# JVBSouza/descriptools

Hardware: AMD Instinct MI355X
Metric: Mcells/s full descriptor chain (higher is better)
Workload: dtype f32; 1 GPU; 16384x16384 synthetic tilted-integer-fBm DEM per GPU, full chain (d8, flowacc, river mask, flowhand/HAND with fused GFI + ln(hl/H), fused slope+TI+MTI, downslope), device-resident; global_dem=16384x16384, river_threshold_cells=524288

## Files before the change

### descriptools_amd/csrc/dt_tiles.hip

```cpp
#include "dt_common.h"
#include "dt_kernels.h"
#include "dt_math.h"

#define TW 64
#define TH 64
#define NT (TW * TH)
#define PS (2 * TW + 2 * (TH - 2))
#define CPT (NT / 256)

#define NX_SINK 0xFFFFu
#define NX_EXIT 0xFFFEu
#define NX_REXIT 0xFFFDu
#define X_NONE 0xFFFFu

__device__ __forceinline__ int dt_slot_of(int ly, int lx) {
  if (ly == 0) return lx;
  if (ly == TH - 1) return TW + lx;
  if (lx == 0) return 2 * TW + (ly - 1);
  if (lx == TW - 1) return 2 * TW + (TH - 2) + (ly - 1);
  return -1;
}
__device__ __forceinline__ void dt_cell_of_slot(int s, int &ly, int &lx) {
  if (s < TW) { ly = 0; lx = s; }
  else if (s < 2 * TW) { ly = TH - 1; lx = s - TW; }
// ... 1201 lines not shown
  if (NODES && threadIdx.x < PS) {
    int ly, lx;
    dt_cell_of_slot(threadIdx.x, ly, lx);
    unsigned long long s = s_st[ly * TW + lx];
    uint32_t ptr = (uint32_t)(s >> 32), nd = (uint32_t)((s >> 16) & 0xFFFFu);
    uint32_t ncf = (uint32_t)(s & 0xFFFFu), nc = ncf & 0x7FFFu;
    uint32_t kind = (ptr >> 12) & 7u, f = ptr & 0xFFFu;
    int fy = (int)f / TW, fx = (int)f % TW;
    unsigned long long o = fht_pack(FHT_DEAD, 0, FHT_DONE);
    if (!(ncf & FHT_DONE)) {
    } else if (kind == K_RIVER) {
      o = fht_pack((uint32_t)((y0 + fy) * w.W + x0 + fx), nd, nc | FHT_DONE);
    } else if (kind == K_EXIT || kind == K_REXIT) {
      int dy, dx;
      dt_d8_delta(s_fdr[f], dy, dx);
      bool diag = dy != 0 && dx != 0;
      uint32_t node = kind == K_EXIT ? dt_node_of(y0 + fy + dy, x0 + fx + dx, tiles_x)
                                     : nnodes + (uint32_t)dt_perim_index(w.H, w.W, y0 + fy, x0 + fx);
      o = fht_pack(node, nd + (diag ? 1u : 0u), nc + (diag ? 0u : 1u));
    }
    nodes[(size_t)tile * PS + threadIdx.x] = o;
  }
  unsigned long long wv[CPT];
  int wide = 0;
#pragma unroll
  for (int j = 0; j < CPT; j++) {
    wv[j] = s_st[threadIdx.x + 256 * j];
    wide |= (((uint32_t)wv[j] & 0x7FFFu) > 255u || ((uint32_t)(wv[j] >> 16) & 0xFFFFu) > 255u) ? 1 : 0;
  }
  wide = __syncthreads_or(wide);
  if (threadIdx.x == 0) cache_wide[tile] = (uint8_t)wide;
  if (wide) {
#pragma unroll
    for (int j = 0; j < CPT; j++) cache[(size_t)tile * NT + threadIdx.x + 256 * j] = wv[j];
  } else {
    uint32_t *c32 = reinterpret_cast<uint32_t *>(cache + (size_t)tile * NT);
#pragma unroll
    for (int j = 0; j < CPT; j++) c32[threadIdx.x + 256 * j] = fh_cache_pack(wv[j]);
  }
  __syncthreads();
}
__global__ __launch_bounds__(256) void k_fh_tile1(const uint8_t *__restrict__ fdr,
                                                 const int8_t *__restrict__ river, DtWin w, int tiles_x,
                                                 uint32_t nnodes, unsigned long long *__restrict__ nodes,
                                                 unsigned long long *__restrict__ cache,
                                                 uint8_t *__restrict__ cache_wide, int only_marked, int ntiles) {
  __shared__ __attribute__((aligned(16))) uint8_t s_fdr[NT];
  __shared__ uint8_t s_halo[2 * (TW + 2) + 2 * TH];
  __shared__ __attribute__((aligned(16))) unsigned long long s_st[NT];
  for (int tile = (int)blockIdx.x; tile < ntiles; tile += (int)gridDim.x) {
    if (only_marked && cache_wide[tile] != 2) continue;
    fh_tile1_tile<true>(s_fdr, s_halo, s_st, tile, fdr, river, w, tiles_x, nnodes, nodes, cache, cache_wide);
  }
}
__global__ __launch_bounds__(256) void k_fh_tile1_marked(const uint8_t *__restrict__ fdr,
                                                        const int8_t *__restrict__ river, DtWin w, int tiles_x,
                                                        uint32_t nnodes, unsigned long long *__restrict__ nodes,
                                                        unsigned long long *__restrict__ cache,
                                                        uint8_t *cache_wide, int ntiles) {
  __shared__ __attribute__((aligned(16))) uint8_t s_fdr[NT];
  __shared__ uint8_t s_halo[2 * (TW + 2) + 2 * TH];
  __shared__ __attribute__((aligned(16))) unsigned long long s_st[NT];
  __shared__ uint8_t s_flag[256];
  const int base = (int)blockIdx.x * 256, mine = base + (int)threadIdx.x;
  const uint8_t flag = mine < ntiles ? cache_wide[mine] : (uint8_t)0;
  s_flag[threadIdx.x] = flag;
  if (!__syncthreads_or(flag == 2)) return;
  for (int i = 0; i < 256; i++)
    if (s_flag[i] == 2)
      fh_tile1_tile<false>(s_fdr, s_halo, s_st, base + i, fdr, river, w, tiles_x, nnodes, nodes, cache, cache_wide);
}

#define FN_CNT 0x3FFFFu
#define FN_DONE 0x40000u
#define FN_LOW 0x7FFFFu
#define FN_OVF 0x20100u
#define FN_PTR_SH 19
__device__ __forceinline__ uint32_t fh_lut_entry(uint32_t code) {
  if (!dt_d8_valid(code)) return 0u;
  int dy, dx;
  dt_d8_delta(code, dy, dx);
  return ((uint32_t)(dy * TW + dx) << FN_PTR_SH) + ((dy != 0 && dx != 0) ? (1u << 9) : 1u);
}
__device__ __forceinline__ bool fh_tile1n_solve(uint8_t *s_fdr, uint32_t *s_w, uint8_t *s_kind, int *s_ovf_p,
                                                const uint32_t *s_lut, const uint32_t (&riv4)[NT / 4 / 256],
                                                const DtWin &w, int y0, int x0, uint2 (&own)[CPT / 2]) {
#define s_ovf (*s_ovf_p)
  const bool interior = dt_tile_interior(w, y0, x0);
  const uint32_t lx0 = (4u * threadIdx.x) & 63u;
#pragma unroll
  for (int u = 0; u < NT / 4 / 256; u++) {
    const int c0 = 4 * (threadIdx.x + 256 * u);
    const uint32_t codes = *reinterpret_cast<const uint32_t *>(&s_fdr[c0]);
    uint32_t wd[4], kinds = 0;
#pragma unroll
    for (int k = 0; k < 4; k++) {
      const int c = c0 + k;
      const uint32_t code = (codes >> (8 * k)) & 0xFFu, cw = (uint32_t)c << FN_PTR_SH;
      const bool is_river = ((riv4[u] >> (8 * k)) & 0xFFu) == 1u;
      uint32_t word = cw | FN_DONE, kind = K_DEAD;
      if (interior) {
        const uint32_t wn = cw + s_lut[code];
        if (code != 0u) {
          if (is_river) {
            kind = K_RIVER;
          } else if (wn & FN_CNT) {
            const bool out = (int32_t)wn < 0 || (((wn >> FN_PTR_SH) & 63u) - (lx0 + (uint32_t)k - 1u)) > 2u;
            if (out) kind = K_EXIT;
            else word = wn;
          }
        }
      } else {
        const int ly = c / TW, lx = c % TW;
        const int y = y0 + ly, x = x0 + lx;
        if (y < w.H && x < w.W && code != 0u) {
          if (is_river) {
            kind = K_RIVER;
          } else if (dt_d8_valid(code)) {
            int dy, dx;
            dt_d8_delta(code, dy, dx);
            uint32_t ny = (uint32_t)(ly + dy), nx = (uint32_t)(lx + dx);
            bool in_tile = ny < (uint32_t)TH && nx < (uint32_t)TW;
            if (dt_in_global(w, y + dy, x + dx)) {
              if (!dt_in_core(w, y + dy, x + dx)) kind = K_REXIT;
              else if (!in_tile) kind = K_EXIT;
              else word = ((ny * TW + nx) << FN_PTR_SH) | ((dy != 0 && dx != 0) ? (1u << 9) : 1u);
            }
          }
        }
      }
      wd[k] = word;
      kinds |= kind << (8 * k);
    }
    *reinterpret_cast<uint4 *>(&s_w[c0]) = make_uint4(wd[0], wd[1], wd[2], wd[3]);
    *reinterpret_cast<uint32_t *>(&s_kind[c0]) = kinds;
  }
  __syncthreads();
  uint2 *s_w2 = reinterpret_cast<uint2 *>(s_w);
#pragma unroll
  for (int j = 0; j < CPT / 2; j++) own[j] = s_w2[threadIdx.x + 256 * j];
  for (int round = 0; round < 13; round++) {
    int changed = 0;
    uint32_t ovf = 0;
#pragma unroll
    for (int j = 0; j < CPT / 2; j++) {
      int c2 = threadIdx.x + 256 * j;
      uint2 v = own[j];
      bool dx = (v.x & FN_DONE) != 0u, dy = (v.y & FN_DONE) != 0u;
      if (dx && dy) continue;
      if (!dx) {
        v.x = s_w[v.x >> FN_PTR_SH] + (v.x & FN_CNT);
        if (!(v.x & (FN_DONE | FN_OVF))) v.x = s_w[v.x >> FN_PTR_SH] + (v.x & FN_CNT);
        ovf |= v.x & FN_OVF;
      }
      if (!dy) {
        v.y = s_w[v.y >> FN_PTR_SH] + (v.y & FN_CNT);
        if (!(v.y & (FN_DONE | FN_OVF))) v.y = s_w[v.y >> FN_PTR_SH] + (v.y & FN_CNT);
        ovf |= v.y & FN_OVF;
      }
      own[j] = v;
      s_w2[c2] = v;
      changed |= ((v.x & v.y & FN_DONE) == 0u) ? 1 : 0;
    }
    if (ovf) s_ovf = 1;
    if (!__syncthreads_or(changed)) break;
    if (s_ovf) break;
  }
  return !s_ovf;
#undef s_ovf
}
__device__ __forceinline__ uint32_t fh_narrow_word(uint32_t v, uint32_t c, const uint8_t *s_kind) {
  uint32_t f = v >> FN_PTR_SH, kind = s_kind[f];
  if (!(v & FN_DONE)) { f = c; kind = K_DEAD; v = 0; }
  return f | (kind << 12) | (((v >> 9) & 0xFFu) << 15) | ((v & 0xFFu) << 23);
}
__device__ __forceinline__ void fh_tile1n_body(uint8_t *s_fdr, uint32_t *s_w, uint8_t *s_kind, int *s_ovf_p,
                                               const uint32_t *s_lut, const uint32_t (&riv4)[NT / 4 / 256],
                                               const DtWin &w, int tile, int tiles_x, int y0, int x0, uint32_t nnodes,
                                               unsigned long long *__restrict__ nodes,
                                               unsigned long long *__restrict__ cache,
                                               uint8_t *__restrict__ cache_wide) {
  uint2 own[CPT / 2];
  if (!fh_tile1n_solve(s_fdr, s_w, s_kind, s_ovf_p, s_lut, riv4, w, y0, x0, own)) {
    if (threadIdx.x == 0) cache_wide[tile] = 2;
    return;
  }
  uint2 *s_w2 = reinterpret_cast<uint2 *>(s_w);
  auto narrow = [&](uint32_t v, uint32_t c) -> uint32_t { return fh_narrow_word(v, c, s_kind); };
#pragma unroll
  for (int j = 0; j < CPT / 2; j++) {
    const int c2 = threadIdx.x + 256 * j;
    s_w2[c2] = make_uint2(narrow(own[j].x, 2u * (uint32_t)c2), narrow(own[j].y, 2u * (uint32_t)c2 + 1u));
  }
  if (threadIdx.x == 0) cache_wide[tile] = 0;
  __syncthreads();
  uint32_t *c32 = reinterpret_cast<uint32_t *>(cache + (size_t)tile * NT);
#pragma unroll
  for (int u = 0; u < NT / 4 / 256; u++) {
    int c = 4 * (threadIdx.x + 256 * u);
    *reinterpret_cast<uint4 *>(c32 + c) = *reinterpret_cast<const uint4 *>(&s_w[c]);
  }
  if (threadIdx.x < PS) {
    int ly, lx;
    dt_cell_of_slot(threadIdx.x, ly, lx);
    unsigned long long sw = fh_cache_unpack(s_w[ly * TW + lx]);
    uint32_t ptr = (uint32_t)(sw >> 32), nd = (uint32_t)((sw >> 16) & 0xFFFFu), nc = (uint32_t)sw & 0x7FFFu;
    uint32_t kind = (ptr >> 12) & 7u, f = ptr & 0xFFFu;
    int fy = (int)f / TW, fx = (int)f % TW;
    unsigned long long o = fht_pack(FHT_DEAD, 0, FHT_DONE);
    if (kind == K_RIVER) {
      o = fht_pack((uint32_t)((y0 + fy) * w.W + x0 + fx), nd, nc | FHT_DONE);
    } else if (kind == K_EXIT || kind == K_REXIT) {
      int dy, dx;
      dt_d8_delta(s_fdr[f], dy, dx);
      bool diag = dy != 0 && dx != 0;
      uint32_t node = kind == K_EXIT ? dt_node_of(y0 + fy + dy, x0 + fx + dx, tiles_x)
                                     : nnodes + (uint32_t)dt_perim_index(w.H, w.W, y0 + fy, x0 + fx);
      o = fht_pack(node, nd + (diag ? 1u : 0u), nc + (diag ? 0u : 1u));
    }
    nodes[(size_t)tile * PS + threadIdx.x] = o;
  }
}

#define NX_RIVER 0xFFFCu
#define FH_SOLVE_LATER 3
__device__ __forceinline__ void fh_walk_body(const uint16_t *s_nxt, const uint8_t *__restrict__ fdr, bool fed, const DtWin &w,
                                             int tile, int tiles_x, int y0, int x0,
                                             unsigned long long *__restrict__ nodes,
                                             uint8_t *__restrict__ cache_wide) {
  constexpr uint32_t PW = TW + 4, NTP = TH * PW;
  if (threadIdx.x == 0) cache_wide[tile] = (uint8_t)FH_SOLVE_LATER;
  if (threadIdx.x >= PS) return;
  unsigned long long o = fht_pack(FHT_DEAD, 0, FHT_DONE);
  if (fed) {
    int ly, lx;
    dt_cell_of_slot(threadIdx.x, ly, lx);
    uint32_t c = (uint32_t)ly * PW + (uint32_t)lx, nc = 0, nd = 0;
    uint32_t n = 0;
    for (int it = 0; it < NT; it++) {
      n = s_nxt[c];
      if (n >= NTP) break;
      const uint32_t d = n > c ? n - c : c - n;
      if (d == 1u || d == PW) nc++;
      else nd++;
      c = n;
    }
    if (n == NX_RIVER || n == NX_EXIT) {
      const int fy = (int)(c / PW), fx = (int)(c % PW);
      const uint32_t code = fdr[(long long)(y0 + fy) * w.ld + x0 + fx];
      if (n == NX_EXIT) {
        int dy, dx;
        dt_d8_delta(code, dy, dx);
        const bool diag = dy != 0 && dx != 0;
        o = fht_pack(dt_node_of(y0 + fy + dy, x0 + fx + dx, tiles_x), nd + (diag ? 1u : 0u), nc + (diag ? 0u : 1u));
      } else if (code != 0u) {
// ... 111 lines not shown
  uint8_t k = (uint8_t)K_DEAD;
  int32_t r = -1;
  float z = DT_NODATA;
  long long a = 0;
  if (ncf & FHT_DONE) {
    if (ptr != FHT_DEAD) {
      k = (uint8_t)K_RIVER;
      r = (int32_t)ptr;
      long long o = (long long)(ptr / (uint32_t)w.W) * w.ld + (ptr % (uint32_t)w.W);
      if (dem) z = dem[o];
      if (acc32) a = (long long)acc32[o];
    }
  } else if (ptr >= nnodes) {
    k = (uint8_t)K_REXIT;
    r = (int32_t)(ptr - nnodes);
  }
  kind[i] = k;
  ref[i] = r;
  nc[i] = (int32_t)(ncf & 0x7FFFu);
  nd[i] = (int32_t)((s >> 16) & 0xFFFFu);
  zr[i] = z;
  ar[i] = a;
}

__global__ __launch_bounds__(256) void k_fh_ghost_set(unsigned long long *__restrict__ nodes, uint32_t nnodes,
                                                     int64_t P, const uint8_t *__restrict__ res_ok,
                                                     const int32_t *__restrict__ res_nc,
                                                     const int32_t *__restrict__ res_nd) {
  int64_t i = (int64_t)blockIdx.x * 256 + threadIdx.x;
  if (i >= P) return;
  unsigned long long o = fht_pack(FHT_DEAD, 0, FHT_DONE);
  if (res_ok[i]) o = fht_pack(FHT_REMOTE | (uint32_t)i, (uint32_t)res_nd[i], (uint32_t)res_nc[i] | FHT_DONE);
  nodes[nnodes + i] = o;
}

struct FhGfi {
  float *gfi, *lnhlh;
  double expo, c0;
  const DtLogEntry *tab;
};
struct FhRemote {
  const long long *gidx;
  const float *zr;
  const long long *ar;
};
template <typename AccT>
struct FhPay;
template <>
struct FhPay<int32_t> {
  unsigned long long v[PS];
  __device__ __forceinline__ void set(int i, float z, int32_t a) {
    v[i] = ((unsigned long long)(uint32_t)a << 32) | (unsigned long long)__float_as_uint(z);
  }
  __device__ __forceinline__ void get(int i, float &z, int32_t &a) const {
    const unsigned long long p = v[i];
    z = __uint_as_float((uint32_t)p);
    a = (int32_t)(uint32_t)(p >> 32);
  }
};
template <>
struct FhPay<long long> {
  long long av[PS];
  float zv[PS];
  __device__ __forceinline__ void set(int i, float z, long long a) {
    av[i] = a;
    zv[i] = z;
  }
  __device__ __forceinline__ void get(int i, float &z, long long &a) const {
    z = zv[i];
    a = av[i];
  }
};

typedef float fh_v4f __attribute__((ext_vector_type(4)));
typedef int fh_v4i __attribute__((ext_vector_type(4)));
__device__ __forceinline__ void fh_store4(float *p, float a, float b, float c, float d) {
  fh_v4f v = {a, b, c, d};
  __builtin_nontemporal_store(v, reinterpret_cast<fh_v4f *>(p));
}
__device__ __forceinline__ void fh_store4(int32_t *p, int32_t a, int32_t b, int32_t c, int32_t d) {
  fh_v4i v = {a, b, c, d};
  __builtin_nontemporal_store(v, reinterpret_cast<fh_v4i *>(p));
}
typedef long long fh_v2l __attribute__((ext_vector_type(2)));
__device__ __forceinline__ void fh_store4(long long *p, long long a, long long b, long long c, long long d) {
  fh_v2l v0 = {a, b}, v1 = {c, d};
  __builtin_nontemporal_store(v0, reinterpret_cast<fh_v2l *>(p));
  __builtin_nontemporal_store(v1, reinterpret_cast<fh_v2l *>(p + 2));
}

struct FhSolveLds {
  uint8_t *fdr;
  uint32_t *w;
  uint8_t *kind;
  uint32_t *lut;
  int *ovf;
  double *term;
};
template <bool RANKED, int VH, typename AccT, bool SOLVE>
__device__ __forceinline__ bool fh_tile3_tile(unsigned long long *s_x, FhPay<AccT> &s_pay, DtLogEntry *s_tab,
                                              const FhSolveLds &L, const int8_t *__restrict__ river, int tile,
                                              const uint8_t *__restrict__ fdr, const float *__restrict__ dem,
                                              const AccT *__restrict__ acc32, const DtWin &w, int tiles_x,
                                              uint32_t nnodes, const unsigned long long *__restrict__ nodes,
                                              const unsigned long long *__restrict__ cache, bool wide,
                                              const FhRemote &rem, double px, float *__restrict__ fdist,
                                              int32_t *__restrict__ idx32, long long *__restrict__ idx64,
                                              float *__restrict__ hand, AccT *__restrict__ a_river,
                                              const FhGfi &G) {
  const int ty = tile / tiles_x, tx = tile - ty * tiles_x;
  const int y0 = ty * TH, x0 = tx * TW;
  const bool vec = x0 + TW <= w.W && (w.ld & 3) == 0 && (!dem || ((uintptr_t)dem & 15) == 0) &&
                   (!fdist || ((uintptr_t)fdist & 15) == 0) && (!idx32 || ((uintptr_t)idx32 & 15) == 0) &&
                   (!idx64 || ((uintptr_t)idx64 & 15) == 0) && (!hand || ((uintptr_t)hand & 15) == 0) &&
                   (!a_river || ((uintptr_t)a_river & 15) == 0) &&
                   (!G.gfi || ((((uintptr_t)G.gfi | (uintptr_t)G.lnhlh | (uintptr_t)acc32) & 15) == 0));
  [[maybe_unused]] auto load_z4 = [&](int u) -> float4 {
    const int c = 4 * (threadIdx.x + 256 * u), y = y0 + c / TW;
    float4 z = make_float4(DT_NODATA, DT_NODATA, DT_NODATA, DT_NODATA);
    if (dem && y < w.H) z = *reinterpret_cast<const float4 *>(dem + (long long)y * w.ld + x0 + c % TW);
    return z;
  };
  [[maybe_unused]] auto load_f4 = [&](int u) -> int4 {
    const int c = 4 * (threadIdx.x + 256 * u), y = y0 + c / TW;
    int4 f = make_int4(0, 0, 0, 0);
    if (G.gfi && y < w.H) f = *reinterpret_cast<const int4 *>(acc32 + (long long)y * w.ld + x0 + c % TW);
    return f;
  };
  float4 z4_first = make_float4(DT_NODATA, DT_NODATA, DT_NODATA, DT_NODATA);
  int4 f4_first = make_int4(0, 0, 0, 0);
  int slot_ly = 0, slot_lx = 0;
  if (threadIdx.x < PS) dt_cell_of_slot(threadIdx.x, slot_ly, slot_lx);
  uint32_t slot_code = 0;
  bool has_river = true;
  if (SOLVE) {
    const uint4 v_fdr = dt_tile_fetch16(fdr, w, y0, x0);
    const uint4 v_riv = dt_tile_fetch16(reinterpret_cast<const uint8_t *>(river), w, y0, x0);
    if (vec) {
      z4_first = load_z4(0);
      f4_first = load_f4(0);
    }
    dt_tile_put16(L.fdr, v_fdr);
    dt_tile_put16(L.kind, v_riv);
    L.lut[threadIdx.x] = fh_lut_entry(threadIdx.x);
    if (threadIdx.x == 0) *L.ovf = 0;
    has_river = __syncthreads_or((v_riv.x | v_riv.y | v_riv.z | v_riv.w) != 0u) != 0;
    if (threadIdx.x < PS) slot_code = L.fdr[slot_ly * TW + slot_lx];
    uint32_t riv4[NT / 4 / 256];
#pragma unroll
    for (int u = 0; u < NT / 4 / 256; u++) riv4[u] = *reinterpret_cast<const uint32_t *>(&L.kind[4 * (threadIdx.x + 256 * u)]);
    uint2 own[CPT / 2];
    if (!fh_tile1n_solve(L.fdr, L.w, L.kind, L.ovf, L.lut, riv4, w, y0, x0, own)) return false;
  }
  auto solved = [&](uint32_t v, int c) -> uint32_t { return fh_narrow_word(v, (uint32_t)c, L.kind); };
  if (threadIdx.x < PS) {
    const int ly = slot_ly, lx = slot_lx;
    int f = ly * TW + lx;
    bool ex, rex;
    if (SOLVE) {
      const uint32_t v = L.w[f];
      const bool self = (v & FN_DONE) != 0u && (v >> FN_PTR_SH) == (uint32_t)f;
      const uint32_t kind = L.kind[f];
      ex = self && kind == K_EXIT;
      rex = self && kind == K_REXIT;
    } else {
      const uint32_t sp = (uint32_t)(fh_cache_get(cache, wide, tile, f) >> 32);
      ex = sp == ((uint32_t)f | (K_EXIT << 12));
      rex = sp == ((uint32_t)f | (K_REXIT << 12));
    }
    unsigned long long o = fht_pack(FHT_DEAD, 0, FHT_DONE);
    float zr = DT_NODATA;
    AccT ar = -100;
    if (ex || rex) {
      int dy, dx;
      dt_d8_delta(SOLVE ? slot_code : (uint32_t)fdr[(long long)(y0 + ly) * w.ld + x0 + lx], dy, dx);
      size_t node = ex ? (size_t)dt_node_of(y0 + ly + dy, x0 + lx + dx, tiles_x)
                       : (size_t)nnodes + (size_t)dt_perim_index(w.H, w.W, y0 + ly, x0 + lx);
      unsigned long long ns = nodes[node];
      uint32_t nptr = (uint32_t)(ns >> 32), nnd = (uint32_t)((ns >> 16) & 0xFFFFu);
      uint32_t nncf = (uint32_t)(ns & 0xFFFFu);
      if (RANKED && !(nncf & FHT_DONE) && nptr >= nnodes && (size_t)nptr != node) {
        unsigned long long gs = nodes[nptr];
        uint32_t gncf = (uint32_t)(gs & 0xFFFFu);
        nnd += (uint32_t)((gs >> 16) & 0xFFFFu);
        const uint32_t cnt = (nncf & 0x7FFFu) + (gncf & 0x7FFFu);
        nptr = (uint32_t)(gs >> 32);
        if ((gncf & FHT_DONE) && nptr != FHT_DEAD && cnt + nnd <= FHT_CAP) nncf = cnt | FHT_DONE;
        else nptr = FHT_DEAD;
      }
      bool diag = dy != 0 && dx != 0;
      if ((nncf & FHT_DONE) && nptr != FHT_DEAD) {
        o = fht_pack(nptr, nnd + (diag ? 1u : 0u), ((nncf & 0x7FFFu) + (diag ? 0u : 1u)) | FHT_DONE);
        if (RANKED && (nptr & FHT_REMOTE)) {
          zr = rem.zr[nptr & ~FHT_REMOTE];
          ar = (AccT)rem.ar[nptr & ~FHT_REMOTE];
        } else {
          long long ro = (long long)(nptr / (uint32_t)w.W) * w.ld + (nptr % (uint32_t)w.W);
          if (dem) zr = dem[ro];
          if (acc32) ar = acc32[ro];
        }
      }
    }
    s_x[threadIdx.x] = o;
    s_pay.set((int)threadIdx.x, zr, ar);
    if (SOLVE && G.gfi) L.term[threadIdx.x] = G.expo * dt_log_sel((double)ar, s_tab);
  }
  const double dcard = px, ddiag = px * sqrt(2.0);
  struct CellOut {
    float fd, h;
    int32_t i32;
    AccT ar;
    long long i64;
  };
  auto solve = [&](unsigned long long s, float z) -> CellOut {
    uint32_t ptr = (uint32_t)(s >> 32), nd = (uint32_t)((s >> 16) & 0xFFFFu);
    uint32_t ncf = (uint32_t)(s & 0xFFFFu), nc = ncf & 0x7FFFu;
    uint32_t kind = (ptr >> 12) & 7u, f = ptr & 0xFFFu;
    bool ok = false;
    uint32_t ridx = 0;
    float pz = 0.0f;
    AccT pa = 0;
    if (ncf & FHT_DONE) {
      if (kind == K_RIVER) {
        ok = true;
        ridx = (uint32_t)((y0 + (int)f / TW) * w.W + x0 + (int)f % TW);
        long long ro = (long long)(y0 + (int)f / TW) * w.ld + x0 + (int)f % TW;
        pz = dem ? dem[ro] : DT_NODATA;
        pa = acc32 ? acc32[ro] : (AccT)-100;
      } else if (kind == K_EXIT || kind == K_REXIT) {
        int slot = dt_slot_of((int)f / TW, (int)f % TW);
        unsigned long long xs = s_x[slot];
        uint32_t xptr = (uint32_t)(xs >> 32);
        if (xptr != FHT_DEAD) {
          nc += (uint32_t)(xs & 0x7FFFu);
          nd += (uint32_t)((xs >> 16) & 0xFFFFu);
          ok = nc + nd <= FHT_CAP;
          ridx = xptr;
          s_pay.get(slot, pz, pa);
        }
      }
    }
    const bool remote = RANKED && ok && (ridx & FHT_REMOTE) != 0u;
    CellOut o;
    o.fd = ok ? (float)(dcard * (double)nc + ddiag * (double)nd) : DT_NODATA;
    o.i32 = (ok && !remote) ? (int32_t)ridx : -100;
    o.i64 = -100;
    if (RANKED && ok) {
      o.i64 = remote ? rem.gidx[ridx & ~FHT_REMOTE]
                     : (long long)(w.gy0 + (int)(ridx / (uint32_t)w.W)) * w.Wg + w.gx0 + (int)(ridx % (uint32_t)w.W);
      o.i32 = (int32_t)o.i64;
    }
    o.h = DT_NODATA;
    if (z != DT_NODATA && ok) {
      o.h = z - pz;
      if (o.h < 0.0f && o.h != DT_NODATA) o.h = 0.0f;
    }
    o.ar = ok ? pa : (AccT)-100;
    return o;
  };
  if constexpr (SOLVE) {
    if (vec) {
      auto cell = [&](auto RIV, uint32_t v, float z, int32_t fown, float &fd, int32_t &i32, float &h, int32_t &ar,
                      float &g, float &l) {
        const bool done = (v & FN_DONE) != 0u;
        const uint32_t e = v >> FN_PTR_SH, ey = e / TW, ex = e % TW;
        const uint32_t kind = L.kind[e];
        const uint32_t slot = ey == 0u ? ex
                                       : (ey == TH - 1u ? TW + ex
                                                        : (ex == 0u ? 2u * TW - 1u + ey : 2u * TW + TH - 3u + ey));
        const unsigned long long xs = s_x[slot];
        uint32_t ridx = (uint32_t)(xs >> 32);
        uint32_t nc = (v & 0xFFu) + (uint32_t)(xs & 0x7FFFu), nd = ((v >> 9) & 0xFFu) + (uint32_t)((xs >> 16) & 0xFFFFu);
        bool ok = done && (kind == K_EXIT || kind == K_REXIT) && ridx != FHT_DEAD && nc + nd <= FHT_CAP;
        float pz;
        int32_t pa;
        s_pay.get((int)slot, pz, pa);
        double term = G.gfi ? L.term[slot] : 0.0;
        if (decltype(RIV)::value) {
          if (done && kind == K_RIVER) {
            ok = true;
            nc = v & 0xFFu;
            nd = (v >> 9) & 0xFFu;
            ridx = (uint32_t)((y0 + (int)ey) * w.W + x0 + (int)ex);
            const long long ro = (long long)(y0 + (int)ey) * w.ld + x0 + (int)ex;
            pz = dem ? dem[ro] : DT_NODATA;
            pa = acc32 ? acc32[ro] : -100;
            if (G.gfi) term = G.expo * dt_log_sel((double)pa, s_tab);
          }
        }
        fd = ok ? (float)(dcard * (double)nc + ddiag * (double)nd) : DT_NODATA;
        i32 = ok ? (int32_t)ridx : -100;
        h = DT_NODATA;
        if (z != DT_NODATA && ok) {
          h = z - pz;
          if (h < 0.0f && h != DT_NODATA) h = 0.0f;
        }
        ar = ok ? pa : -100;
        if (G.gfi) dt_gfi_both_cell_term(h, term, fown, G.expo, G.c0, s_tab, g, l);
      };
      auto stream = [&](auto RIV) {
        float4 z4 = z4_first;
        int4 f4 = f4_first;
#pragma unroll 1
        for (int u = 0; u < NT / 4 / 256; u++) {
          const int c = 4 * (threadIdx.x + 256 * u);
          const int y = y0 + c / TW;
          const long long o = (long long)y * w.ld + x0 + c % TW;
          const uint4 v = *reinterpret_cast<const uint4 *>(&L.w[c]);
          const float4 z4_cur = z4;
          int4 f4_cur = f4;
          if (u + 1 < NT / 4 / 256) {
            z4 = load_z4(u + 1);
            f4 = load_f4(u + 1);
          }
          if (u == 0) __syncthreads();
          asm volatile("" : "+v"(f4_cur.x), "+v"(f4_cur.y), "+v"(f4_cur.z), "+v"(f4_cur.w));
          if (y >= w.H) continue;
          float4 fd, hh, g, l;
          int4 ix, ar;
          cell(RIV, v.x, z4_cur.x, f4_cur.x, fd.x, ix.x, hh.x, ar.x, g.x, l.x);
          __builtin_amdgcn_sched_barrier(0);
          cell(RIV, v.y, z4_cur.y, f4_cur.y, fd.y, ix.y, hh.y, ar.y, g.y, l.y);
          __builtin_amdgcn_sched_barrier(0);
          cell(RIV, v.z, z4_cur.z, f4_cur.z, fd.z, ix.z, hh.z, ar.z, g.z, l.z);
          __builtin_amdgcn_sched_barrier(0);
          cell(RIV, v.w, z4_cur.w, f4_cur.w, fd.w, ix.w, hh.w, ar.w, g.w, l.w);
          if (fdist) fh_store4(fdist + o, fd.x, fd.y, fd.z, fd.w);
          if (idx32) fh_store4(idx32 + o, ix.x, ix.y, ix.z, ix.w);
          if (hand) fh_store4(hand + o, hh.x, hh.y, hh.z, hh.w);
          if (a_river) fh_store4(a_river + o, ar.x, ar.y, ar.z, ar.w);
          if (G.gfi) {
            fh_store4(G.gfi + o, g.x, g.y, g.z, g.w);
            fh_store4(G.lnhlh + o, l.x, l.y, l.z, l.w);
          }
          __builtin_amdgcn_sched_barrier(0);
        }
      };
      if (has_river) stream(std::integral_constant<bool, true>{});
      else stream(std::integral_constant<bool, false>{});
      return true;
    }
  }
  if (vec) {
    constexpr int VPT = NT / 4 / 256;
#pragma unroll 1
    for (int h = 0; h < VPT / VH; h++) {
      uint4 wa[VH], wb[VH];
      float4 z4[VH];
#pragma unroll
      for (int u = 0; u < VH; u++) {
        int c = 4 * (threadIdx.x + 256 * (h * VH + u));
        if (wide) {
          const uint4 *cp = reinterpret_cast<const uint4 *>(cache + (size_t)tile * NT + c);
          wa[u] = cp[0];
          wb[u] = cp[1];
        } else {
          uint4 v;
          if (SOLVE) {
            v = *reinterpret_cast<const uint4 *>(&L.w[c]);
            v = make_uint4(solved(v.x, c), solved(v.y, c + 1), solved(v.z, c + 2), solved(v.w, c + 3));
          } else {
            v = *reinterpret_cast<const uint4 *>(reinterpret_cast<const uint32_t *>(cache + (size_t)tile * NT) + c);
          }
          unsigned long long a = fh_cache_unpack(v.x), b2 = fh_cache_unpack(v.y), c2 = fh_cache_unpack(v.z),
                             d2 = fh_cache_unpack(v.w);
          wa[u] = make_uint4((uint32_t)a, (uint32_t)(a >> 32), (uint32_t)b2, (uint32_t)(b2 >> 32));
          wb[u] = make_uint4((uint32_t)c2, (uint32_t)(c2 >> 32), (uint32_t)d2, (uint32_t)(d2 >> 32));
        }
        int y = y0 + c / TW;
        z4[u] = make_float4(DT_NODATA, DT_NODATA, DT_NODATA, DT_NODATA);
        if (dem && y < w.H) z4[u] = *reinterpret_cast<const float4 *>(dem + (long long)y * w.ld + x0 + c % TW);
      }
      if (h == 0) __syncthreads();
#pragma unroll
      for (int u = 0; u < VH; u++) {
        int c = 4 * (threadIdx.x + 256 * (h * VH + u));
        int y = y0 + c / TW;
        if (y >= w.H) continue;
        long long o = (long long)y * w.ld + x0 + c % TW;
        CellOut r0 = solve(((unsigned long long)wa[u].y << 32) | wa[u].x, z4[u].x);
        CellOut r1 = solve(((unsigned long long)wa[u].w << 32) | wa[u].z, z4[u].y);
        CellOut r2 = solve(((unsigned long long)wb[u].y << 32) | wb[u].x, z4[u].z);
        CellOut r3 = solve(((unsigned long long)wb[u].w << 32) | wb[u].z, z4[u].w);
        if (fdist) fh_store4(fdist + o, r0.fd, r1.fd, r2.fd, r3.fd);
        if (idx32) fh_store4(idx32 + o, r0.i32, r1.i32, r2.i32, r3.i32);
        if (RANKED && idx64) {
          *reinterpret_cast<longlong2 *>(idx64 + o) = make_longlong2(r0.i64, r1.i64);
          *reinterpret_cast<longlong2 *>(idx64 + o + 2) = make_longlong2(r2.i64, r3.i64);
        }
        if (hand) fh_store4(hand + o, r0.h, r1.h, r2.h, r3.h);
        if (a_river) fh_store4(a_river + o, r0.ar, r1.ar, r2.ar, r3.ar);
        if (G.gfi) {
          AccT fx, fy, fz, fw;
          if (sizeof(AccT) == 8) {
            const longlong2 fa = *reinterpret_cast<const longlong2 *>(acc32 + o);
            const longlong2 fb = *reinterpret_cast<const longlong2 *>(acc32 + o + 2);
            fx = (AccT)fa.x; fy = (AccT)fa.y; fz = (AccT)fb.x; fw = (AccT)fb.y;
          } else {
            const int4 f = *reinterpret_cast<const int4 *>(acc32 + o);
            fx = (AccT)f.x; fy = (AccT)f.y; fz = (AccT)f.z; fw = (AccT)f.w;
          }
          float4 g, l;
          dt_gfi_both_cell(r0.h, r0.ar, fx, G.expo, G.c0, s_tab, g.x, l.x);
          __builtin_amdgcn_sched_barrier(0);
          dt_gfi_both_cell(r1.h, r1.ar, fy, G.expo, G.c0, s_tab, g.y, l.y);
          __builtin_amdgcn_sched_barrier(0);
          dt_gfi_both_cell(r2.h, r2.ar, fz, G.expo, G.c0, s_tab, g.z, l.z);
          __builtin_amdgcn_sched_barrier(0);
          dt_gfi_both_cell(r3.h, r3.ar, fw, G.expo, G.c0, s_tab, g.w, l.w);
          fh_store4(G.gfi + o, g.x, g.y, g.z, g.w);
          fh_store4(G.lnhlh + o, l.x, l.y, l.z, l.w);
        }
        __builtin_amdgcn_sched_barrier(0);
      }
    }
    return true;
  }
  __syncthreads();
#pragma unroll 1
  for (int j = 0; j < CPT; j++) {
    int c = threadIdx.x + 256 * j;
    int y = y0 + c / TW, x = x0 + c % TW;
    if (y >= w.H || x >= w.W) continue;
    long long o = (long long)y * w.ld + x;
    CellOut r = solve(SOLVE ? fh_cache_unpack(solved(L.w[c], c)) : fh_cache_get(cache, wide, tile, c),
                      dem ? dem[o] : DT_NODATA);
    if (fdist) fdist[o] = r.fd;
    if (idx32) idx32[o] = r.i32;
    if (RANKED && idx64) idx64[o] = r.i64;
    if (hand) hand[o] = r.h;
    if (a_river) a_river[o] = r.ar;
    if (G.gfi) {
      float g, l;
      dt_gfi_both_cell(r.h, r.ar, acc32[o], G.expo, G.c0, s_tab, g, l);
      G.gfi[o] = g;
      G.lnhlh[o] = l;
    }
  }
  return true;
}

template <bool RANKED, int VH, int MINW, typename AccT>
__global__ __launch_bounds__(256, MINW) void k_fh_tile3(const uint8_t *__restrict__ fdr,
                                                 const float *__restrict__ dem,
                                                 const AccT *__restrict__ acc32, DtWin w, int tiles_x,
                                                 uint32_t nnodes, const unsigned long long *__restrict__ nodes,
                                                 const unsigned long long *__restrict__ cache,
                                                 const uint8_t *__restrict__ cache_wide,
                                                 FhRemote rem, double px, float *__restrict__ fdist,
                                                 int32_t *__restrict__ idx32, long long *__restrict__ idx64,
                                                 float *__restrict__ hand, AccT *__restrict__ a_river,
                                                 FhGfi G) {
  __shared__ unsigned long long s_x[PS];
  __shared__ FhPay<AccT> s_pay;
  __shared__ DtLogEntry s_tab[DT_LOGTAB_N];
  if (G.gfi) dt_math_stage(G.tab, s_tab);
  const int tile = dt_tile_of_block((int)blockIdx.x, (int)gridDim.x);
  const bool wide = cache_wide[tile] != 0;
  fh_tile3_tile<RANKED, VH, AccT, false>(s_x, s_pay, s_tab, FhSolveLds{}, nullptr, tile, fdr, dem, acc32, w, tiles_x,
                                         nnodes, nodes, cache, wide, rem, px, fdist, idx32, idx64, hand, a_river, G);
}

__global__ __launch_bounds__(256, 5) void k_fh_tile3_solve(const uint8_t *__restrict__ fdr,
                                                          const int8_t *__restrict__ river,
                                                          const float *__restrict__ dem,
                                                          const int32_t *__restrict__ acc32, DtWin w, int tiles_x,
                                                          uint32_t nnodes,
                                                          const unsigned long long *__restrict__ nodes,
                                                          uint8_t *__restrict__ cache_wide, double px,
                                                          float *__restrict__ fdist, int32_t *__restrict__ idx32,
                                                          float *__restrict__ hand, int32_t *__restrict__ a_river,
                                                          FhGfi G) {
  __shared__ unsigned long long s_x[PS];
  __shared__ FhPay<int32_t> s_pay;
  __shared__ DtLogEntry s_tab[DT_LOGTAB_N];
  __shared__ __attribute__((aligned(16))) uint8_t s_fdr[NT];
  __shared__ __attribute__((aligned(16))) uint32_t s_w[NT];
  __shared__ __attribute__((aligned(16))) uint8_t s_kind[NT];
  __shared__ uint32_t s_lut[256];
  __shared__ int s_ovf;
  if (G.gfi) dt_math_stage(G.tab, s_tab);
  const int tile = dt_tile_of_block((int)blockIdx.x, (int)gridDim.x);
  const bool ok = fh_tile3_tile<false, 1, int32_t, true>(
      s_x, s_pay, s_tab, FhSolveLds{s_fdr, s_w, s_kind, s_lut, &s_ovf, reinterpret_cast<double *>(s_fdr)}, river, tile, fdr, dem, acc32, w, tiles_x, nnodes,
      nodes, nullptr, false, FhRemote{nullptr, nullptr, nullptr}, px, fdist, idx32, nullptr, hand, a_river, G);
  if (!ok && threadIdx.x == 0) cache_wide[tile] = 2;
}

__global__ __launch_bounds__(256) void k_fh_tile3_marked(const uint8_t *__restrict__ fdr,
                                                           const float *__restrict__ dem,
                                                           const int32_t *__restrict__ acc32, DtWin w, int tiles_x,
                                                           uint32_t nnodes,
                                                           const unsigned long long *__restrict__ nodes,
                                                           const unsigned long long *__restrict__ cache,
                                                           const uint8_t *__restrict__ cache_wide, int ntiles,
                                                           double px, float *__restrict__ fdist,
                                                           int32_t *__restrict__ idx32, float *__restrict__ hand,
                                                           int32_t *__restrict__ a_river, FhGfi G) {
  __shared__ unsigned long long s_x[PS];
  __shared__ FhPay<int32_t> s_pay;
  __shared__ DtLogEntry s_tab[DT_LOGTAB_N];
  __shared__ uint8_t s_flag[256];
  const int base = (int)blockIdx.x * 256, mine = base + (int)threadIdx.x;
  const uint8_t flag = mine < ntiles ? cache_wide[mine] : (uint8_t)FH_SOLVE_LATER;
  s_flag[threadIdx.x] = flag;
  if (!__syncthreads_or(flag != FH_SOLVE_LATER)) return;
  if (G.gfi) dt_math_stage(G.tab, s_tab);
  for (int i = 0; i < 256; i++) {
    if (s_flag[i] == FH_SOLVE_LATER) continue;
    fh_tile3_tile<false, 1, int32_t, false>(s_x, s_pay, s_tab, FhSolveLds{}, nullptr, base + i, fdr, dem, acc32, w,
                                            tiles_x, nnodes, nodes, cache, s_flag[i] != 0, FhRemote{nullptr, nullptr, nullptr},
                                            px, fdist, idx32, nullptr, hand, a_river, G);
    __syncthreads();
  }
}
__global__ __launch_bounds__(256) void k_fh_mark_all(uint8_t *__restrict__ cache_wide, int ntiles) {
  const int t = (int)blockIdx.x * 256 + (int)threadIdx.x;
  if (t < ntiles && cache_wide[t] == FH_SOLVE_LATER) cache_wide[t] = 2;
}

struct FhScratch {
  unsigned long long *nodes, *cache;
  int *flags;
  uint8_t *cache_wide;
  int64_t nnodes, ntiles, P;
  int tiles_x;
  size_t bytes;
};
static FhScratch fh_layout(const DtWin &w, void *scratch) {
  FhScratch f;
  f.tiles_x = (w.W + TW - 1) / TW;
  f.ntiles = (int64_t)f.tiles_x * ((w.H + TH - 1) / TH);
  f.nnodes = f.ntiles * PS;
  f.P = dt_perim_count(w.H, w.W);
  DtCarver c(scratch);
  f.nodes = c.take<unsigned long long>((size_t)f.nnodes + (size_t)f.P);
  f.cache = c.take<unsigned long long>((size_t)f.ntiles * NT);
  f.flags = (int *)c.raw(256);
  f.cache_wide = c.take<uint8_t>((size_t)f.ntiles);
  f.bytes = c.bytes();
  return f;
}
size_t dt_flowhand_tiled_scratch(int64_t H, int64_t W) { return fh_layout(dt_full_window(H, W), nullptr).bytes; }

static int fh_local_tail(hipStream_t s, const DtWin &w, const uint8_t *fdr, const int8_t *river, const FhScratch &f,
                         bool walked = false) {
  dim3 gt((unsigned)f.ntiles), b(256);
  if (!walked)
    hipLaunchKernelGGL(k_fh_tile1, dim3(gt.x < 2048u ? gt.x : 2048u), b, 0, s, fdr, river, w, f.tiles_x,
                       (uint32_t)f.nnodes, f.nodes, f.cache, f.cache_wide, 1, (int)f.ntiles);
  hipLaunchKernelGGL(k_fh_ghost_init, dim3((unsigned)((f.P + 255) / 256)), b, 0, s, f.nodes, (uint32_t)f.nnodes, f.P);
  DT_HIP(hipMemsetAsync(f.flags, 0, 64, s));
  dim3 gj(dt_capped_grid(f.nnodes + f.P, 4096));
  for (int r = 0; r < 8; r++)
    hipLaunchKernelGGL(k_fh_node_jump, gj, b, 0, s, f.nodes, f.nnodes + f.P, f.flags, r, 3);
  return DT_OK;
}

int dt_launch_fh_local(hipStream_t s, const DtWin &w, const uint8_t *fdr, const int8_t *river, void *scratch,
                       size_t scratch_bytes) {
  if (w.H == 0 || w.W == 0) return DT_OK;
  FhScratch f = fh_layout(w, scratch);
  DT_REQUIRE(scratch_bytes >= f.bytes, "scratch too small");
  DT_REQUIRE(f.nnodes + f.P < 0x7FFFFFF0ll, "raster too large for one device tile");
  hipLaunchKernelGGL(k_fh_tile1n, dim3((unsigned)f.ntiles), dim3(256), 0, s, fdr, river, w, f.tiles_x,
                     (uint32_t)f.nnodes, f.nodes, f.cache, f.cache_wide);
  return fh_local_tail(s, w, fdr, river, f);
// ... 427 lines not shown
```

Before: 37990 Mcells/s.

## Shrink LDS footprint of HAND solve kernel to raise occupancy

Packs the per-cell kind array to 2 bits and the river mask to bits, and overlays s_x and the LUT/river bits onto existing shared buffers. Launch bounds rise from 5 to 6 blocks per CU. It also moves the boundary-slot lookup into a hook that runs right after solve setup, and computes store addresses from scalar row bases plus per-lane offsets. The GFI computation is deferred until after the main stores, and the acc32 load is issued per iteration instead of being prefetched. The intent is more concurrent blocks and fewer address VGPRs. The risks are extra bit-unpacking work, register spilling under the tighter bound, and LDS aliasing hazards from the overlays.

```diff
diff --git a/descriptools_amd/csrc/dt_tiles.hip b/descriptools_amd/csrc/dt_tiles.hip
--- a/descriptools_amd/csrc/dt_tiles.hip
+++ b/descriptools_amd/csrc/dt_tiles.hip
@@ -1307,9 +1307,19 @@
   dt_d8_delta(code, dy, dx);
   return ((uint32_t)(dy * TW + dx) << FN_PTR_SH) + ((dy != 0 && dx != 0) ? (1u << 9) : 1u);
 }
+struct FhNoHook {
+  __device__ __forceinline__ void operator()() const {}
+};
+template <bool PACK>
+__device__ __forceinline__ uint32_t fh_kind_get(const uint8_t *s_kind, uint32_t c) {
+  if (PACK) return (((uint32_t)s_kind[c >> 2] >> (2u * (c & 3u))) & 3u) + 1u;
+  return s_kind[c];
+}
+template <bool PACK = false, typename Hook = FhNoHook>
 __device__ __forceinline__ bool fh_tile1n_solve(uint8_t *s_fdr, uint32_t *s_w, uint8_t *s_kind, int *s_ovf_p,
                                                 const uint32_t *s_lut, const uint32_t (&riv4)[NT / 4 / 256],
-                                                const DtWin &w, int y0, int x0, uint2 (&own)[CPT / 2]) {
+                                                const DtWin &w, int y0, int x0, uint2 (&own)[CPT / 2],
+                                                Hook after_setup = Hook{}) {
 #define s_ovf (*s_ovf_p)
   const bool interior = dt_tile_interior(w, y0, x0);
   const uint32_t lx0 = (4u * threadIdx.x) & 63u;
@@ -1322,7 +1332,7 @@
     for (int k = 0; k < 4; k++) {
       const int c = c0 + k;
       const uint32_t code = (codes >> (8 * k)) & 0xFFu, cw = (uint32_t)c << FN_PTR_SH;
-      const bool is_river = ((riv4[u] >> (8 * k)) & 0xFFu) == 1u;
+      const bool is_river = PACK ? ((riv4[u] >> k) & 1u) != 0u : ((riv4[u] >> (8 * k)) & 0xFFu) == 1u;
       uint32_t word = cw | FN_DONE, kind = K_DEAD;
       if (interior) {
         const uint32_t wn = cw + s_lut[code];
@@ -1355,12 +1365,14 @@
         }
       }
       wd[k] = word;
-      kinds |= kind << (8 * k);
+      kinds |= PACK ? (kind - 1u) << (2 * k) : kind << (8 * k);
     }
     *reinterpret_cast<uint4 *>(&s_w[c0]) = make_uint4(wd[0], wd[1], wd[2], wd[3]);
-    *reinterpret_cast<uint32_t *>(&s_kind[c0]) = kinds;
+    if (PACK) s_kind[c0 >> 2] = (uint8_t)kinds;
+    else *reinterpret_cast<uint32_t *>(&s_kind[c0]) = kinds;
   }
   __syncthreads();
+  after_setup();
   uint2 *s_w2 = reinterpret_cast<uint2 *>(s_w);
 #pragma unroll
   for (int j = 0; j < CPT / 2; j++) own[j] = s_w2[threadIdx.x + 256 * j];
@@ -1394,8 +1406,9 @@
   return !s_ovf;
 #undef s_ovf
 }
+template <bool PACK = false>
 __device__ __forceinline__ uint32_t fh_narrow_word(uint32_t v, uint32_t c, const uint8_t *s_kind) {
-  uint32_t f = v >> FN_PTR_SH, kind = s_kind[f];
+  uint32_t f = v >> FN_PTR_SH, kind = fh_kind_get<PACK>(s_kind, f);
   if (!(v & FN_DONE)) { f = c; kind = K_DEAD; v = 0; }
   return f | (kind << 12) | (((v >> 9) & 0xFFu) << 15) | ((v & 0xFFu) << 23);
 }
@@ -1673,6 +1686,15 @@
   fh_v4i v = {a, b, c, d};
   __builtin_nontemporal_store(v, reinterpret_cast<fh_v4i *>(p));
 }
+typedef __attribute__((address_space(1))) char fh_gchar;
+__device__ __forceinline__ void fh_store4(fh_gchar *p, float a, float b, float c, float d) {
+  fh_v4f v = {a, b, c, d};
+  __builtin_nontemporal_store(v, (__attribute__((address_space(1))) fh_v4f *)p);
+}
+__device__ __forceinline__ void fh_store4(fh_gchar *p, int32_t a, int32_t b, int32_t c, int32_t d) {
+  fh_v4i v = {a, b, c, d};
+  __builtin_nontemporal_store(v, (__attribute__((address_space(1))) fh_v4i *)p);
+}
 typedef long long fh_v2l __attribute__((ext_vector_type(2)));
 __device__ __forceinline__ void fh_store4(long long *p, long long a, long long b, long long c, long long d) {
   fh_v2l v0 = {a, b}, v1 = {c, d};
@@ -1685,9 +1707,15 @@
   uint32_t *w;
   uint8_t *kind;
   uint32_t *lut;
+  uint16_t *rivb;
   int *ovf;
   double *term;
 };
+__device__ __forceinline__ uint32_t fh_riv_bits(uint32_t x) {
+  const uint32_t y = x ^ 0x01010101u;
+  const uint32_t z = ~(((y & 0x7F7F7F7Fu) + 0x7F7F7F7Fu) | y | 0x7F7F7F7Fu);
+  return (((z >> 7) * 0x00204081u) >> 21) & 0xFu;
+}
 template <bool RANKED, int VH, typename AccT, bool SOLVE>
 __device__ __forceinline__ bool fh_tile3_tile(unsigned long long *s_x, FhPay<AccT> &s_pay, DtLogEntry *s_tab,
                                               const FhSolveLds &L, const int8_t *__restrict__ river, int tile,
@@ -1705,60 +1733,45 @@
                    (!fdist || ((uintptr_t)fdist & 15) == 0) && (!idx32 || ((uintptr_t)idx32 & 15) == 0) &&
                    (!idx64 || ((uintptr_t)idx64 & 15) == 0) && (!hand || ((uintptr_t)hand & 15) == 0) &&
                    (!a_river || ((uintptr_t)a_river & 15) == 0) &&
-                   (!G.gfi || ((((uintptr_t)G.gfi | (uintptr_t)G.lnhlh | (uintptr_t)acc32) & 15) == 0));
+                   (!G.gfi || ((((uintptr_t)G.gfi | (uintptr_t)G.lnhlh | (uintptr_t)acc32) & 15) == 0)) &&
+                   (!SOLVE || w.ld <= (1ll << 24));
+  [[maybe_unused]] const uint32_t lane_b = 4u * ((threadIdx.x >> 4) * (uint32_t)w.ld + ((4u * threadIdx.x) & 63u));
+  [[maybe_unused]] auto at = [&](const void *base, int u) -> fh_gchar * {
+    const uintptr_t row = (uintptr_t)base + (uintptr_t)(((long long)(y0 + 16 * u) * w.ld + x0) * 4);
+    const uintptr_t srow = ((uintptr_t)(uint32_t)__builtin_amdgcn_readfirstlane((uint32_t)(row >> 32)) << 32) |
+                           (uintptr_t)(uint32_t)__builtin_amdgcn_readfirstlane((uint32_t)row);
+    uint32_t lb = lane_b;
+    asm volatile("" : "+v"(lb));
+    return (fh_gchar *)srow + lb;
+  };
   [[maybe_unused]] auto load_z4 = [&](int u) -> float4 {
-    const int c = 4 * (threadIdx.x + 256 * u), y = y0 + c / TW;
+    const int y = y0 + 16 * u + (int)(threadIdx.x >> 4);
     float4 z = make_float4(DT_NODATA, DT_NODATA, DT_NODATA, DT_NODATA);
-    if (dem && y < w.H) z = *reinterpret_cast<const float4 *>(dem + (long long)y * w.ld + x0 + c % TW);
+    if (dem && y < w.H) {
+      const fh_v4f v = *(const __attribute__((address_space(1))) fh_v4f *)at(dem, u);
+      z = make_float4(v.x, v.y, v.z, v.w);
+    }
     return z;
   };
   [[maybe_unused]] auto load_f4 = [&](int u) -> int4 {
-    const int c = 4 * (threadIdx.x + 256 * u), y = y0 + c / TW;
+    const int y = y0 + 16 * u + (int)(threadIdx.x >> 4);
     int4 f = make_int4(0, 0, 0, 0);
-    if (G.gfi && y < w.H) f = *reinterpret_cast<const int4 *>(acc32 + (long long)y * w.ld + x0 + c % TW);
+    if (G.gfi && y < w.H) {
+      const fh_v4i v = *(const __attribute__((address_space(1))) fh_v4i *)at(acc32, u);
+      f = make_int4(v.x, v.y, v.z, v.w);
+    }
     return f;
   };
   float4 z4_first = make_float4(DT_NODATA, DT_NODATA, DT_NODATA, DT_NODATA);
-  int4 f4_first = make_int4(0, 0, 0, 0);
   int slot_ly = 0, slot_lx = 0;
   if (threadIdx.x < PS) dt_cell_of_slot(threadIdx.x, slot_ly, slot_lx);
   uint32_t slot_code = 0;
   bool has_river = true;
-  if (SOLVE) {
-    const uint4 v_fdr = dt_tile_fetch16(fdr, w, y0, x0);
-    const uint4 v_riv = dt_tile_fetch16(reinterpret_cast<const uint8_t *>(river), w, y0, x0);
-    if (vec) {
-      z4_first = load_z4(0);
-      f4_first = load_f4(0);
-    }
-    dt_tile_put16(L.fdr, v_fdr);
-    dt_tile_put16(L.kind, v_riv);
-    L.lut[threadIdx.x] = fh_lut_entry(threadIdx.x);
-    if (threadIdx.x == 0) *L.ovf = 0;
-    has_river = __syncthreads_or((v_riv.x | v_riv.y | v_riv.z | v_riv.w) != 0u) != 0;
-    if (threadIdx.x < PS) slot_code = L.fdr[slot_ly * TW + slot_lx];
-    uint32_t riv4[NT / 4 / 256];
-#pragma unroll
-    for (int u = 0; u < NT / 4 / 256; u++) riv4[u] = *reinterpret_cast<const uint32_t *>(&L.kind[4 * (threadIdx.x + 256 * u)]);
-    uint2 own[CPT / 2];
-    if (!fh_tile1n_solve(L.fdr, L.w, L.kind, L.ovf, L.lut, riv4, w, y0, x0, own)) return false;
-  }
-  auto solved = [&](uint32_t v, int c) -> uint32_t { return fh_narrow_word(v, (uint32_t)c, L.kind); };
-  if (threadIdx.x < PS) {
+  unsigned long long slot_o = fht_pack(FHT_DEAD, 0, FHT_DONE);
+  float slot_zr = DT_NODATA;
+  AccT slot_ar = -100;
+  auto lookup = [&](bool ex, bool rex) {
     const int ly = slot_ly, lx = slot_lx;
-    int f = ly * TW + lx;
-    bool ex, rex;
-    if (SOLVE) {
-      const uint32_t v = L.w[f];
-      const bool self = (v & FN_DONE) != 0u && (v >> FN_PTR_SH) == (uint32_t)f;
-      const uint32_t kind = L.kind[f];
-      ex = self && kind == K_EXIT;
-      rex = self && kind == K_REXIT;
-    } else {
-      const uint32_t sp = (uint32_t)(fh_cache_get(cache, wide, tile, f) >> 32);
-      ex = sp == ((uint32_t)f | (K_EXIT << 12));
-      rex = sp == ((uint32_t)f | (K_REXIT << 12));
-    }
     unsigned long long o = fht_pack(FHT_DEAD, 0, FHT_DONE);
     float zr = DT_NODATA;
     AccT ar = -100;
@@ -1792,6 +1805,46 @@
         }
       }
     }
+    slot_o = o;
+    slot_zr = zr;
+    slot_ar = ar;
+  };
+  if (SOLVE) {
+    const uint4 v_fdr = dt_tile_fetch16(fdr, w, y0, x0);
+    const uint4 v_riv = dt_tile_fetch16(reinterpret_cast<const uint8_t *>(river), w, y0, x0);
+    if (vec) z4_first = load_z4(0);
+    dt_tile_put16(L.fdr, v_fdr);
+    L.rivb[threadIdx.x] = (uint16_t)(fh_riv_bits(v_riv.x) | (fh_riv_bits(v_riv.y) << 4) | (fh_riv_bits(v_riv.z) << 8) |
+                                     (fh_riv_bits(v_riv.w) << 12));
+    L.lut[threadIdx.x] = fh_lut_entry(threadIdx.x);
+    if (threadIdx.x == 0) *L.ovf = 0;
+    has_river = __syncthreads_or((v_riv.x | v_riv.y | v_riv.z | v_riv.w) != 0u) != 0;
+    if (threadIdx.x < PS) slot_code = L.fdr[slot_ly * TW + slot_lx];
+    uint32_t riv4[NT / 4 / 256];
+#pragma unroll
+    for (int u = 0; u < NT / 4 / 256; u++)
+      riv4[u] = ((uint32_t)L.rivb[(threadIdx.x >> 2) + 64 * u] >> (4u * (threadIdx.x & 3u))) & 0xFu;
+    uint2 own[CPT / 2];
+    auto early = [&]() {
+      if (threadIdx.x < PS) {
+        const uint32_t f = (uint32_t)(slot_ly * TW + slot_lx), v = L.w[f];
+        const bool self = (v & FN_DONE) != 0u && (v >> FN_PTR_SH) == f;
+        const uint32_t kind = fh_kind_get<true>(L.kind, f);
+        lookup(self && kind == K_EXIT, self && kind == K_REXIT);
+      }
+    };
+    if (!fh_tile1n_solve<true>(L.fdr, L.w, L.kind, L.ovf, L.lut, riv4, w, y0, x0, own, early)) return false;
+  }
+  auto solved = [&](uint32_t v, int c) -> uint32_t { return fh_narrow_word<SOLVE>(v, (uint32_t)c, L.kind); };
+  if (threadIdx.x < PS) {
+    if (!SOLVE) {
+      const int f = slot_ly * TW + slot_lx;
+      const uint32_t sp = (uint32_t)(fh_cache_get(cache, wide, tile, f) >> 32);
+      lookup(sp == ((uint32_t)f | (K_EXIT << 12)), sp == ((uint32_t)f | (K_REXIT << 12)));
+    }
+    const unsigned long long o = slot_o;
+    const float zr = slot_zr;
+    const AccT ar = slot_ar;
     s_x[threadIdx.x] = o;
     s_pay.set((int)threadIdx.x, zr, ar);
     if (SOLVE && G.gfi) L.term[threadIdx.x] = G.expo * dt_log_sel((double)ar, s_tab);
@@ -1851,11 +1904,10 @@
   };
   if constexpr (SOLVE) {
     if (vec) {
-      auto cell = [&](auto RIV, uint32_t v, float z, int32_t fown, float &fd, int32_t &i32, float &h, int32_t &ar,
-                      float &g, float &l) {
+      auto cell = [&](auto RIV, uint32_t v, float z, float &fd, int32_t &i32, float &h, int32_t &ar, double &term) {
         const bool done = (v & FN_DONE) != 0u;
         const uint32_t e = v >> FN_PTR_SH, ey = e / TW, ex = e % TW;
-        const uint32_t kind = L.kind[e];
+        const uint32_t kind = fh_kind_get<true>(L.kind, e);
         const uint32_t slot = ey == 0u ? ex
                                        : (ey == TH - 1u ? TW + ex
                                                         : (ex == 0u ? 2u * TW - 1u + ey : 2u * TW + TH - 3u + ey));
@@ -1866,7 +1918,7 @@
         float pz;
         int32_t pa;
         s_pay.get((int)slot, pz, pa);
-        double term = G.gfi ? L.term[slot] : 0.0;
+        term = G.gfi ? L.term[slot] : 0.0;
         if (decltype(RIV)::value) {
           if (done && kind == K_RIVER) {
             ok = true;
@@ -1887,42 +1939,46 @@
           if (h < 0.0f && h != DT_NODATA) h = 0.0f;
         }
         ar = ok ? pa : -100;
-        if (G.gfi) dt_gfi_both_cell_term(h, term, fown, G.expo, G.c0, s_tab, g, l);
       };
       auto stream = [&](auto RIV) {
         float4 z4 = z4_first;
-        int4 f4 = f4_first;
 #pragma unroll 1
         for (int u = 0; u < NT / 4 / 256; u++) {
           const int c = 4 * (threadIdx.x + 256 * u);
           const int y = y0 + c / TW;
-          const long long o = (long long)y * w.ld + x0 + c % TW;
           const uint4 v = *reinterpret_cast<const uint4 *>(&L.w[c]);
           const float4 z4_cur = z4;
-          int4 f4_cur = f4;
-          if (u + 1 < NT / 4 / 256) {
-            z4 = load_z4(u + 1);
-            f4 = load_f4(u + 1);
-          }
+          int4 f4_cur = load_f4(u);
+          if (u + 1 < NT / 4 / 256) z4 = load_z4(u + 1);
           if (u == 0) __syncthreads();
+          if (y >= w.H) continue;
+          float4 fd, hh;
+          int4 ix, ar;
+          double tm[4];
+          cell(RIV, v.x, z4_cur.x, fd.x, ix.x, hh.x, ar.x, tm[0]);
+          __builtin_amdgcn_sched_barrier(0);
+          cell(RIV, v.y, z4_cur.y, fd.y, ix.y, hh.y, ar.y, tm[1]);
+          __builtin_amdgcn_sched_barrier(0);
+          cell(RIV, v.z, z4_cur.z, fd.z, ix.z, hh.z, ar.z, tm[2]);
+          __builtin_amdgcn_sched_barrier(0);
+          cell(RIV, v.w, z4_cur.w, fd.w, ix.w, hh.w, ar.w, tm[3]);
+          if (fdist) fh_store4(at(fdist, u), fd.x, fd.y, fd.z, fd.w);
+          if (idx32) fh_store4(at(idx32, u), ix.x, ix.y, ix.z, ix.w);
+          if (hand) fh_store4(at(hand, u), hh.x, hh.y, hh.z, hh.w);
+          if (a_river) fh_store4(at(a_river, u), ar.x, ar.y, ar.z, ar.w);
           asm volatile("" : "+v"(f4_cur.x), "+v"(f4_cur.y), "+v"(f4_cur.z), "+v"(f4_cur.w));
-          if (y >= w.H) continue;
-          float4 fd, hh, g, l;
-          int4 ix, ar;
-          cell(RIV, v.x, z4_cur.x, f4_cur.x, fd.x, ix.x, hh.x, ar.x, g.x, l.x);
-          __builtin_amdgcn_sched_barrier(0);
-          cell(RIV, v.y, z4_cur.y, f4_cur.y, fd.y, ix.y, hh.y, ar.y, g.y, l.y);
-          __builtin_amdgcn_sched_barrier(0);
-          cell(RIV, v.z, z4_cur.z, f4_cur.z, fd.z, ix.z, hh.z, ar.z, g.z, l.z);
-          __builtin_amdgcn_sched_barrier(0);
-          cell(RIV, v.w, z4_cur.w, f4_cur.w, fd.w, ix.w, hh.w, ar.w, g.w, l.w);
-          if (fdist) fh_store4(fdist + o, fd.x, fd.y, fd.z, fd.w);
-          if (idx32) fh_store4(idx32 + o, ix.x, ix.y, ix.z, ix.w);
-          if (hand) fh_store4(hand + o, hh.x, hh.y, hh.z, hh.w);
-          if (a_river) fh_store4(a_river + o, ar.x, ar.y, ar.z, ar.w);
           if (G.gfi) {
-            fh_store4(G.gfi + o, g.x, g.y, g.z, g.w);
-            fh_store4(G.lnhlh + o, l.x, l.y, l.z, l.w);
+            float4 g, l;
+            __builtin_amdgcn_sched_barrier(0);
+            dt_gfi_both_cell_term(hh.x, tm[0], f4_cur.x, G.expo, G.c0, s_tab, g.x, l.x);
+            __builtin_amdgcn_sched_barrier(0);
+            dt_gfi_both_cell_term(hh.y, tm[1], f4_cur.y, G.expo, G.c0, s_tab, g.y, l.y);
+            __builtin_amdgcn_sched_barrier(0);
+            dt_gfi_both_cell_term(hh.z, tm[2], f4_cur.z, G.expo, G.c0, s_tab, g.z, l.z);
+            __builtin_amdgcn_sched_barrier(0);
+            dt_gfi_both_cell_term(hh.w, tm[3], f4_cur.w, G.expo, G.c0, s_tab, g.w, l.w);
+            fh_store4(at(G.gfi, u), g.x, g.y, g.z, g.w);
+            fh_store4(at(G.lnhlh, u), l.x, l.y, l.z, l.w);
           }
           __builtin_amdgcn_sched_barrier(0);
         }
@@ -2052,7 +2108,7 @@
                                          nnodes, nodes, cache, wide, rem, px, fdist, idx32, idx64, hand, a_river, G);
 }
 
-__global__ __launch_bounds__(256, 5) void k_fh_tile3_solve(const uint8_t *__restrict__ fdr,
+__global__ __launch_bounds__(256, 6) void k_fh_tile3_solve(const uint8_t *__restrict__ fdr,
                                                           const int8_t *__restrict__ river,
                                                           const float *__restrict__ dem,
                                                           const int32_t *__restrict__ acc32, DtWin w, int tiles_x,
@@ -2062,18 +2118,22 @@
                                                           float *__restrict__ fdist, int32_t *__restrict__ idx32,
                                                           float *__restrict__ hand, int32_t *__restrict__ a_river,
                                                           FhGfi G) {
-  __shared__ unsigned long long s_x[PS];
-  __shared__ FhPay<int32_t> s_pay;
   __shared__ DtLogEntry s_tab[DT_LOGTAB_N];
   __shared__ __attribute__((aligned(16))) uint8_t s_fdr[NT];
   __shared__ __attribute__((aligned(16))) uint32_t s_w[NT];
-  __shared__ __attribute__((aligned(16))) uint8_t s_kind[NT];
-  __shared__ uint32_t s_lut[256];
+  __shared__ __attribute__((aligned(16))) uint8_t s_kind[NT / 4];
+  __shared__ __attribute__((aligned(16))) FhPay<int32_t> s_pay;
   __shared__ int s_ovf;
+  static_assert(2 * PS * 8 <= NT && 256 * 4 + 256 * 2 <= sizeof(FhPay<int32_t>), "the overlays fit");
+  unsigned long long *s_x = reinterpret_cast<unsigned long long *>(s_fdr) + PS;
+  uint32_t *s_lut = reinterpret_cast<uint32_t *>(&s_pay);
   if (G.gfi) dt_math_stage(G.tab, s_tab);
   const int tile = dt_tile_of_block((int)blockIdx.x, (int)gridDim.x);
   const bool ok = fh_tile3_tile<false, 1, int32_t, true>(
-      s_x, s_pay, s_tab, FhSolveLds{s_fdr, s_w, s_kind, s_lut, &s_ovf, reinterpret_cast<double *>(s_fdr)}, river, tile, fdr, dem, acc32, w, tiles_x, nnodes,
+      s_x, s_pay, s_tab,
+      FhSolveLds{s_fdr, s_w, s_kind, s_lut, reinterpret_cast<uint16_t *>(s_lut + 256), &s_ovf,
+                 reinterpret_cast<double *>(s_fdr)},
+      river, tile, fdr, dem, acc32, w, tiles_x, nnodes,
       nodes, nullptr, false, FhRemote{nullptr, nullptr, nullptr}, px, fdist, idx32, nullptr, hand, a_river, G);
   if (!ok && threadIdx.x == 0) cache_wide[tile] = 2;
 }
```

Result: no change. 37870 Mcells/s (-0.3%).
